# AITRICS/Medical_Tri_Modal_Pilot

Hardware: AMD Instinct MI355X
Metric: tri-modal training samples/s (fwd+bwd+AdamW step, per-GPU batch 64) (higher is better)
Workload: dtype bf16; 1 GPU; BASELINE configs[1]: vslt_img_txt tri_mbt_vsltcls, 6 layers, d_model 256, batch 64/GPU, TIE-len 1000 (N_v=1005), 224x224 CXR, 128-tok text, dropout 0.1, mbt-only-vslt 1, imgtxt-time 1; global_batch=64, parallelism=dp1

## Files before the change

### include/mtmp.h

```cpp
#ifndef MTMP_H
#define MTMP_H
#include <stdint.h>
#ifdef __cplusplus
extern "C" {
#endif

#define MTMP_F32 0
#define MTMP_BF16 1

int mtmp_abi_version(void);
const char* mtmp_last_error(void);

int mtmp_attn_fwd(int dtype, const void* q, const void* k, const void* v, void* o, const void* res, void* o_res,
                  float* lse, const int32_t* kv_len, const float* key_norms, int B, int N, int H, int ld_qkv, int ld_o,
                  float scale, void* stream);
int mtmp_attn_fwd_grouped(int dtype, int n, const void* const* q, const void* const* k, const void* const* v, void* const* o,
                          const void* const* res, void* const* o_res, float* const* lse, const int32_t* const* kv_len,
                          const int32_t* const* row_start, const float* const* key_norms, const int* N, const int* ld_qkv,
                          const int* ld_o, int B, int H, float scale, void* stream);
int mtmp_attn_bwd_grouped(int dtype, int n, const void* const* q, const void* const* k, const void* const* v,
                          const void* const* o, const void* const* d_o, const float* const* lse, const int32_t* const* kv_len,
                          const int32_t* const* row_start, void* const* dq, void* const* dk, void* const* dv,
                          float* const* delta_ws, const int* N, const int* ld_qkv, const int* ld_o, const int* ld_do,
                          const int* ld_dqkv, int B, int H, float scale, void* stream);
int mtmp_attn_cls_fwd(int dtype, const void* q, const void* k, const void* v, int ld_qkv, const void* res, int ld_res, void* o_cls,
                      void* r1_cls, float* lse, const int32_t* kv_len, const int32_t* row_start, int B, int N, int H, int cls_tok,
                      float scale, void* stream);
int mtmp_attn_cls_bwd(int dtype, const void* q, const void* k, const void* v, int ld_qkv, const void* o_cls, const void* d_o,
                      const float* lse, const int32_t* kv_len, const int32_t* row_start, void* dq, void* dk, void* dv, int ld_dqkv,
                      int B, int N, int H, int cls_tok, float scale, void* stream);
long long mtmp_key_norms_floats(long long rows, int H);
int mtmp_key_norms(int dtype, const void* k, float* out, long long rows, int H, int ld, void* stream);

int mtmp_attn_bwd(int dtype, const void* q, const void* k, const void* v, const void* o, const void* d_o,
                  const float* lse, const int32_t* kv_len, void* dq, void* dk, void* dv, float* delta_ws, int B,
                  int N, int H, int ld_qkv, int ld_o, int ld_do, int ld_dqkv, float scale, void* stream);

int mtmp_ln_gemm(int dtype, const void* x, const float* gamma, const float* beta, const void* w, const float* bias,
                 void* y, void* xn, float* stats, int M, int N, int ldx, int ldy, float eps, int relu, float drop_p,
                 unsigned seed, const unsigned* seed_dev, void* stream);

int mtmp_ln_gemm_qkv(int dtype, const void* x, const float* gamma, const float* beta, const void* w, const float* bias,
                     void* y, void* xn, float* stats, float* key_norms, int M, int ldx, float eps, void* stream);

int mtmp_gemm_nt(int dtype, const void* a, const void* w, const float* bias, const void* res, void* y, int M, int N,
                 int K, int lda, int ldy, int ldr, int act, float drop_p, unsigned seed, const unsigned* seed_dev,
                 const void* gate, float gate_scale, const float* row_scale, int rows_per_scale, void* stream);

long long mtmp_sign_bits_bytes(int M, int N);
int mtmp_ln_gemm_signs(int dtype, const void* x, const float* gamma, const float* beta, const void* w, const float* bias,
                       void* y, void* xn, float* stats, int M, int N, int ldx, int ldy, float eps, float drop_p,
                       unsigned seed, const unsigned* seed_dev, void* signs, void* stream);
int mtmp_gemm_nt_signs(int dtype, const void* a, const void* w, void* y, int M, int N, int lda, int ldy,
                       const void* signs, float gate_scale, void* stream);
int mtmp_gemm_nt_signs_drop(int dtype, const void* a, const void* w, void* y, int M, int N, int lda, int ldy,
                            const void* signs, float gate_scale, float drop_p, unsigned seed, const unsigned* seed_dev,
                            void* a_out, void* stream);

long long mtmp_gemm_tn_ws_floats(int M, int N, int K);
int mtmp_gemm_tn(int dtype, const void* dy, const void* x, float* dw, float* db, float* ws, int M, int N, int K,
                 int ldy, int ldx, void* stream);
int mtmp_gemm_tn_live(int dtype, const void* dy, const void* x, float* dw, float* db, float* ws, int M, int N, int K,
                      int ldy, int ldx, const int32_t* rows_live, void* stream);

int mtmp_dropout_bwd(int dtype, const void* g_in, void* g_out, long long n, unsigned seed, const unsigned* seed_dev,
                     float p, void* stream);

int mtmp_ln_bwd_ws_floats(int M);
int mtmp_ln_bwd(int dtype, const void* z, int ldz, const float* stats, const float* gamma, const void* dy,
                const void* d_res, int ldr, void* dz, float* dgamma_dbeta, float* ws, int M, float eps, void* stream);

int mtmp_gemm_lnbwd_ws_floats(int M);
int mtmp_gemm_lnbwd(int dtype, const void* dy, const void* wt, const void* z, int ldz, const float* stats,
                    const float* gamma, const void* d_res, int ldr, void* dz, float* dgamma_dbeta, float* ws, int M,
                    int K, int ldy, float eps, void* stream);

int mtmp_tie_embed_fwd(int dtype, const float* events, const float* params, const float* ftab, void* out, int n,
                       void* stream);
int mtmp_tie_bwd_ws_floats(int n);
int mtmp_tie_embed_bwd(int dtype, const float* events, const float* params, const void* d_out, float* grads,
                       float* ws, int n, void* stream);

int mtmp_time_embed_fwd(int dtype, const float* events, const float* params, const float* ftab, void* out, int n,
// ... 167 lines not shown
```

### medical_tri_modal_pilot_amd/_lib.py

```python
import ctypes
import os
from ctypes import c_char_p, c_float, c_int, c_longlong, c_uint, c_void_p

_HERE = os.path.dirname(os.path.abspath(__file__))
LIB_PATH = os.environ.get("MTMP_LIB", os.path.join(_HERE, "libmtmp_hip.so"))

F32, BF16 = 0, 1

SIGNATURES = {
    "mtmp_abi_version": (c_int, []),
    "mtmp_last_error": (c_char_p, []),
    "mtmp_attn_fwd": (c_int, [c_int] + [c_void_p] * 9 + [c_int] * 5 + [c_float, c_void_p]),
    "mtmp_attn_cls_fwd": (c_int, [c_int] + [c_void_p] * 3 + [c_int, c_void_p, c_int] + [c_void_p] * 5 + [c_int] * 4 + [c_float, c_void_p]),
    "mtmp_attn_cls_bwd": (c_int, [c_int] + [c_void_p] * 3 + [c_int] + [c_void_p] * 8 + [c_int] * 5 + [c_float, c_void_p]),
    "mtmp_attn_fwd_grouped": (c_int, [c_int, c_int] + [c_void_p] * 13 + [c_int, c_int, c_float, c_void_p]),
    "mtmp_attn_bwd_grouped": (c_int, [c_int, c_int] + [c_void_p] * 17 + [c_int, c_int, c_float, c_void_p]),
    "mtmp_key_norms_floats": (c_longlong, [c_longlong, c_int]),
    "mtmp_key_norms": (c_int, [c_int, c_void_p, c_void_p, c_longlong, c_int, c_int, c_void_p]),
    "mtmp_attn_bwd": (c_int, [c_int] + [c_void_p] * 11 + [c_int] * 7 + [c_float, c_void_p]),
    "mtmp_ln_gemm": (c_int, [c_int] + [c_void_p] * 8 + [c_int] * 4 + [c_float, c_int, c_float, c_uint, c_void_p, c_void_p]),
    "mtmp_ln_gemm_qkv": (c_int, [c_int] + [c_void_p] * 9 + [c_int, c_int, c_float, c_void_p]),
    "mtmp_gemm_nt": (c_int, [c_int] + [c_void_p] * 5 + [c_int] * 7 + [c_float, c_uint, c_void_p, c_void_p, c_float, c_void_p, c_int,
                             c_void_p]),
    "mtmp_gemm_nt_live": (c_int, [c_int] + [c_void_p] * 5 + [c_int] * 7 + [c_float, c_uint, c_void_p, c_void_p, c_float, c_void_p, c_int,
                             c_void_p, c_void_p]),
    "mtmp_sign_bits_bytes": (c_longlong, [c_int, c_int]),
    "mtmp_ln_gemm_signs": (c_int, [c_int] + [c_void_p] * 8 + [c_int] * 4 + [c_float, c_float, c_uint, c_void_p, c_void_p, c_void_p]),
    "mtmp_gemm_nt_signs": (c_int, [c_int] + [c_void_p] * 3 + [c_int] * 4 + [c_void_p, c_float, c_void_p]),
    "mtmp_gemm_nt_signs_drop": (c_int, [c_int] + [c_void_p] * 3 + [c_int] * 4 + [c_void_p, c_float, c_float, c_uint, c_void_p,
                                                                                   c_void_p, c_void_p]),
    "mtmp_ln_gemm_qkv_grouped": (c_int, [c_int, c_int] + [c_void_p] * 11 + [c_float, c_void_p, c_void_p]),
    "mtmp_ln_gemm_signs_grouped": (c_int, [c_int, c_int] + [c_void_p] * 10 + [c_int, c_void_p, c_float, c_float, c_void_p, c_void_p,
                                                                                   c_void_p, c_void_p]),
    "mtmp_gemm_nt_grouped": (c_int, [c_int, c_int] + [c_void_p] * 6 + [c_int, c_int] + [c_void_p] * 3 + [c_int, c_float, c_void_p,
                                                                                                       c_void_p, c_void_p, c_void_p]),
    "mtmp_gemm_nt_signs_drop_grouped": (c_int, [c_int, c_int] + [c_void_p] * 4 + [c_int, c_void_p, c_void_p, c_float, c_float,
                                                                                  c_void_p, c_void_p, c_void_p, c_void_p, c_void_p]),
    "mtmp_gemm_lnbwd_grouped": (c_int, [c_int, c_int] + [c_void_p] * 11 + [c_int, c_void_p, c_float, c_void_p, c_void_p]),
    "mtmp_gemm_tn_group_plan": (c_int, [c_int, c_void_p, c_int, c_int, c_void_p]),
    "mtmp_gemm_tn_grouped": (c_int, [c_int, c_int] + [c_void_p] * 4 + [c_int, c_int] + [c_void_p] * 4 + [c_void_p]),
    "mtmp_gemm_tn_slab_rows": (c_int, [c_int] * 4),
    "mtmp_gemm_lnbwd_slab_rows": (c_int, [c_int]),
    "mtmp_reduce_batch": (c_int, [c_void_p] * 6 + [c_int, c_void_p]),
    "mtmp_reduce_scatter": (c_int, [c_void_p] * 5 + [c_int, c_void_p]),
    "mtmp_stream_input_slab_rows": (c_int, [c_int]),
    "mtmp_stream_input_bwd_partials": (c_int, [c_int] + [c_void_p] * 7 + [c_int] * 3 + [c_float, c_uint, c_void_p, c_void_p, c_void_p, c_void_p]),
    "mtmp_stream_input_bwd_grouped": (c_int, [c_int, c_int] + [c_void_p] * 18),
    "mtmp_stream_input_fwd_add": (c_int, [c_int] + [c_void_p] * 8 + [c_int] * 3 + [c_float, c_float, c_uint, c_void_p, c_void_p, c_void_p, c_void_p, c_int, c_void_p]),
    "mtmp_token_sums": (c_int, [c_int, c_int] + [c_void_p] * 5),
    "mtmp_tie_bwd_slab_rows": (c_int, [c_int]),
    "mtmp_tie_time_embed_bwd_partials": (c_int, [c_int, c_void_p, c_int, c_void_p, c_int, c_int] + [c_void_p] * 6),
    "mtmp_publish_scalar": (c_int, [c_void_p, c_void_p, c_void_p]),
    "mtmp_copy_batch": (c_int, [c_void_p] * 4 + [c_int, c_void_p]),
    "mtmp_stream_lengths": (c_int, [c_void_p] * 4 + [c_int] * 3 + [c_void_p]),
    "mtmp_row_starts": (c_int, [c_void_p, c_void_p, c_int, c_int, c_void_p]),
    "mtmp_image_slots": (c_int, [c_void_p, c_int, c_void_p, c_int, c_int, c_void_p]),
    "mtmp_transpose_batch": (c_int, [c_int, c_void_p, c_void_p, c_void_p, c_void_p, c_int, c_void_p]),
    "mtmp_layernorm_rows": (c_int, [c_int] + [c_void_p] * 4 + [c_longlong, c_int, c_float, c_int, c_int, c_int, c_void_p]),
    "mtmp_layernorm_rows_live": (c_int, [c_int] + [c_void_p] * 4 + [c_longlong, c_int, c_float, c_int, c_int, c_int, c_void_p, c_void_p]),
    "mtmp_swin_window_attn": (c_int, [c_int] + [c_void_p] * 3 + [c_int] * 6 + [c_float, c_void_p]),
    "mtmp_swin_window_attn_live": (c_int, [c_int] + [c_void_p] * 3 + [c_int] * 6 + [c_float, c_void_p, c_void_p]),
    "mtmp_layernorm_rows_bwd_slab_rows": (c_int, [c_longlong, c_int]),
    "mtmp_layernorm_rows_bwd": (c_int, [c_int] + [c_void_p] * 5 + [c_longlong, c_int, c_float, c_void_p]),
    "mtmp_gelu_fwd": (c_int, [c_int, c_void_p, c_void_p, c_longlong, c_void_p]),
    "mtmp_gelu_bwd": (c_int, [c_int, c_void_p, c_void_p, c_void_p, c_longlong, c_void_p]),
    "mtmp_swin_window_attn_bwd": (c_int, [c_int] + [c_void_p] * 5 + [c_int] * 6 + [c_float, c_void_p]),
    "mtmp_swin_window_attn_pad": (c_int, [c_int] + [c_void_p] * 4 + [c_int] * 6 + [c_float, c_void_p, c_void_p]),
# ... 68 lines not shown
```

### medical_tri_modal_pilot_amd/ops.py

```python
import contextlib
import ctypes
from typing import Optional

import torch

from . import _lib, tuning
from ._lib import BF16, F32, call

LN_EPS = 1e-6
N_HEAD, D_MODEL, D_HEAD = 4, 256, 64


def _dt(t: torch.Tensor) -> int:
    if t.dtype == torch.float32:
        return F32
    if t.dtype == torch.bfloat16:
        return BF16
    raise TypeError(f"libmtmp_hip kernels take float32 or bfloat16, got {t.dtype}")


def _p(t: Optional[torch.Tensor], byte_offset: int = 0):
    return None if t is None else ctypes.c_void_p(t.data_ptr() + byte_offset)


# ... 1218 lines not shown
        dqkv = attn_bwd(qkv, o, dr1.view(B, N, D), lse, kv_len).view(M, 3 * D)
    else:
        dqkv = attn_bwd_grouped([qkv], [o], [_packed_full(dr1, B, N)], [lse], [kv_len], [pack])[0].view(M, 3 * D)[:live]
    dwqkv, dbqkv = gemm_tn(dqkv, xn1, out=(sink.wqkv, sink.bqkv) if direct else None, defer=red)
    dz, dg1, db1 = gemm_lnbwd(dqkv, wqkvt, z.view(M, D)[:live], st1, g1, d_res2d=dr1, gb_out=sink.gb1 if direct else None, defer=red)
    if late is not None and red:
        late.append((red, sink if direct else None))
    else:
        if red:
            reduce_batch(red)
        if direct:
            sink.flat.mark_ready(sink.idx)
    dz = dz.view(B, N, D) if pack is None else _packed_full(dz, B, N)
    if direct:
        return dz, None
    grads = (dg1, db1, dwqkv[:D], dbqkv[:D], dwqkv[D:2 * D], dbqkv[D:2 * D], dwqkv[2 * D:], dbqkv[2 * D:],
             dg2, db2, dw1, dc1, dw2, dc2)
    return dz, grads


def attn_cls_fwd(qkv, z, kv_len, pack, cls_tok):
    _gpu(qkv, z)
    B, N, _ = qkv.shape
    es = qkv.element_size()
    o = torch.empty(B, D_MODEL, dtype=qkv.dtype, device=qkv.device)
    r1 = torch.empty_like(o)
    lse = torch.empty(B, N_HEAD, dtype=torch.float32, device=qkv.device)
    call("mtmp_attn_cls_fwd", _dt(qkv), _p(qkv), _p(qkv, D_MODEL * es), _p(qkv, 2 * D_MODEL * es), qkv.stride(1), _p(z), z.stride(1),
         _p(o), _p(r1), _p(lse), _p(kv_len), _p(pack), B, N, N_HEAD, int(cls_tok), D_HEAD ** -0.5, _stream())
    return o, r1, lse


def attn_cls_bwd(qkv, o_cls, d_o, lse, kv_len, pack, cls_tok):
    _gpu(qkv, o_cls, d_o)
    B, N, _ = qkv.shape
    es = qkv.element_size()
    dqkv = torch.empty_like(qkv)
    call("mtmp_attn_cls_bwd", _dt(qkv), _p(qkv), _p(qkv, D_MODEL * es), _p(qkv, 2 * D_MODEL * es), qkv.stride(1), _p(o_cls), _p(_c(d_o)),
         _p(lse), _p(kv_len), _p(pack), _p(dqkv), _p(dqkv, D_MODEL * es), _p(dqkv, 2 * D_MODEL * es), dqkv.stride(1), B, N, N_HEAD,
         int(cls_tok), D_HEAD ** -0.5, _stream())
    return dqkv


_cls_rows_cache = {}


def _cls_rows(B, N, cls_tok, dev):
    key = (B, N, cls_tok, dev.type, dev.index)
    if key not in _cls_rows_cache:
        _cls_rows_cache[key] = (torch.arange(B, dtype=torch.int64) * N + cls_tok).to(dev)
    return _cls_rows_cache[key]


def cls_layer_forward(z, kv_len, P, fused, drop_p, seeds, pack, cls_tok):
    B, N, D = z.shape
    g1, b1, g2, b2, c1, c2 = P[0], P[1], P[8], P[9], P[11], P[13]
    wqkv, bqkv, w1c, w2c, w2t, wqkvt, w1t = fused
    z2 = z.view(B * N, D)
    if pack is not None:
        qkv, xn1, st1 = (t[0] for t in ln_gemm_qkv_grouped([z2], [g1], [b1], [wqkv], [bqkv], [pack])[:3])
    else:
        qkv, xn1, st1 = ln_gemm(z2, g1, b1, wqkv, bqkv, 3 * D)
    qkv = qkv.view(B, N, 3 * D)
    o_cls, r1, lse = attn_cls_fwd(qkv, z, kv_len, pack, cls_tok)
    h, xn2, st2, hsign = ln_gemm(r1, g2, b2, w1c, c1, 4 * D, relu=True, drop_p=drop_p, seed=seeds[0], want_signs=True)
    out = gemm_nt(h, w2c, c2, res2d=r1, drop_p=drop_p, seed=seeds[1])
    rows = pack[:B] if pack is not None else _cls_rows(B, N, cls_tok, z.device)
    return out, (z, kv_len, g1, g2, wqkvt, w1t, w2t, xn1, st1, qkv, o_cls, lse, r1, xn2, st2, h, drop_p, seeds, hsign, pack, rows, cls_tok)


def cls_layer_backward(saved, d_cls, sink=None, late=None):
    z, kv_len, g1, g2, wqkvt, w1t, w2t, xn1, st1, qkv, o_cls, lse, r1, xn2, st2, h, p, seeds, hsign, pack, rows, cls_tok = saved
    B, N, D = z.shape
    M = B * N
    d_out = _c(d_cls).to(z.dtype)
    direct = sink is not None and sink.usable()
    red = [] if tuning.DEFER_REDUCTIONS else None
    if hsign is not None and p > 0 and tuning.FOLD_DROPOUT_BWD:
        dh, dy2 = gemm_nt_signs(d_out, w2t, hsign, 1.0 / (1.0 - p), drop_p=p, seed=seeds[1])
    else:
        dy2 = dropout_bwd(d_out, seeds[1], p) if p > 0 else d_out
        dh = gemm_nt_signs(dy2, w2t, hsign, 1.0 / (1.0 - p)) if hsign is not None else gemm_nt(dy2, w2t, gate=h, gate_scale=1.0 / (1.0 - p))
    dw2, dc2 = gemm_tn(dy2, h, out=(sink.w2, sink.c2) if direct else None, defer=red)
    dw1, dc1 = gemm_tn(dh, xn2, out=(sink.w1, sink.c1) if direct else None, defer=red)
    dr1, dg2, db2 = gemm_lnbwd(dh, w1t, r1, st2, g2, d_res2d=d_out, gb_out=sink.gb2 if direct else None, defer=red)
    dqkv = attn_cls_bwd(qkv, o_cls, dr1, lse, kv_len, pack, cls_tok).view(M, 3 * D)
    z2 = z.view(M, D)
    if pack is not None:
        dwqkv, dbqkv = gemm_tn_grouped([dqkv], [xn1], [(sink.wqkv, sink.bqkv) if direct else None], [red], [pack])[0]
        dz, dg1, db1 = gemm_lnbwd_grouped([dqkv], [wqkvt], [z2], [st1], [g1], [None], [sink.gb1 if direct else None], [red], [pack])[0]
    else:
        dwqkv, dbqkv = gemm_tn(dqkv, xn1, out=(sink.wqkv, sink.bqkv) if direct else None, defer=red)
        dz, dg1, db1 = gemm_lnbwd(dqkv, wqkvt, z2, st1, g1, d_res2d=None, gb_out=sink.gb1 if direct else None, defer=red)
    (dz[cls_tok:] if pack is not None else dz).index_add_(0, rows, dr1)
    if late is not None and red:
        late.append((red, sink if direct else None))
    else:
        if red:
            reduce_batch(red)
        if direct:
            sink.flat.mark_ready(sink.idx)
    if direct:
        return dz.view(B, N, D), None
    grads = (dg1, db1, dwqkv[:D], dbqkv[:D], dwqkv[D:2 * D], dbqkv[D:2 * D], dwqkv[2 * D:], dbqkv[2 * D:],
             dg2, db2, dw1, dc1, dw2, dc2)
    return dz.view(B, N, D), grads




def grouped_ok(z) -> bool:
    return tuning.GROUPED_LAUNCHES and z.dtype == torch.bfloat16


def layer_forward_grouped(zs, kv_lens, Ps, fuseds, drop_p, seeds, packs=None, ffn_rows=None):
    n = len(zs)
    B, D = zs[0].shape[0], D_MODEL
    Ns = [z.shape[1] for z in zs]
    packs = [None] * n if packs is None else list(packs)
    z2 = [z.view(B * N, D) for z, N in zip(zs, Ns)]
    qkv, xn1, st1, knorm = ln_gemm_qkv_grouped(z2, [P[0] for P in Ps], [P[1] for P in Ps], [f[0] for f in fuseds], [f[1] for f in fuseds],
                                               packs)
    qkv = [q.view(B, N, 3 * D) for q, N in zip(qkv, Ns)]
    o, r1, lse = attn_fwd_grouped(qkv, kv_lens, list(zs), knorm, packs)
    R = ffn_rows
    if R is not None:
        if any(pk is not None for pk in packs) or any(N < R for N in Ns):
            raise ValueError("ffn_rows: padded streams of at least that many rows")
        r1_2 = [r[:, :R].reshape(B * R, D) for r in r1]
    else:
        r1_2 = [r.view(B * N, D) for r, N in zip(r1, Ns)]
    h, xn2, st2, hsign = ln_gemm_signs_grouped(r1_2, [P[8] for P in Ps], [P[9] for P in Ps], [f[2] for f in fuseds],
                                               [P[11] for P in Ps], 4 * D, drop_p, [sd[0] for sd in seeds], packs)
    out = gemm_nt_grouped(h, [f[3] for f in fuseds], [P[13] for P in Ps], r1_2, drop_p, [sd[1] for sd in seeds], packs)
    if R is not None:
        full = [torch.zeros(B, N, D, dtype=zs[0].dtype, device=zs[0].device) for N in Ns]
        for f_, o_ in zip(full, out):
            f_[:, :R] = o_.view(B, R, D)
        out = full
    saved = [(zs[i], kv_lens[i], Ps[i][0], Ps[i][8], fuseds[i][5], fuseds[i][6], fuseds[i][4], xn1[i], st1[i], qkv[i], o[i], lse[i],
              r1_2[i] if R is not None else r1[i], xn2[i], st2[i], h[i], drop_p, seeds[i], hsign[i], packs[i], R) for i in range(n)]
    return [out[i].view(B, Ns[i], D) for i in range(n)], saved


def layer_backward_grouped(saveds, d_outs, sinks, late):
    n = len(saveds)
    B, D = saveds[0][0].shape[0], D_MODEL
    Ns = [sv[0].shape[1] for sv in saveds]
    Ms = [B * N for N in Ns]
    p = saveds[0][16]
    d_out = [d.view(M, D) for d, M in zip(d_outs, Ms)]
    direct = [sk is not None and sk.usable() for sk in sinks]
    reds = [[] for _ in range(n)]
    col = lambda k: [sv[k] for sv in saveds]
    z, g1, g2, wqkvt, w1t, w2t, xn1, st1, qkv, o, lse, r1, xn2, st2, h, hsign = (col(0), col(2), col(3), col(4), col(5), col(6), col(7),
                                                                              col(8), col(9), col(10), col(11), col(12), col(13),
                                                                              col(14), col(15), col(18))
    kv = col(1)
    seeds = col(17)
# ... 328 lines not shown
```

### medical_tri_modal_pilot_amd/tuning.py

```python

FOLD_DROPOUT_BWD = True
DEFER_REDUCTIONS = True
LATE_REDUCTIONS = False
GROUPED_LAUNCHES = True
GROUP_MODE = "small"
FFN_ROWS_BEFORE_LAST = True
STREAM_ISSUE_ORDER_FWD = (0, 1, 2)
STREAM_ISSUE_ORDER_BWD = (0, 1, 2)
PREFORK_IMAGE_ENCODER = True
INPUT_NODE_ORDER = "long_last"
FUSED_INPUT_TAIL = True
```

Baseline: 8433 samples/s.

## Replace CLS-layer QKV GEMM with algebraic per-row LN score kernels

Result: no change. 8519 samples/s, median of 6 (+1.0%).

```diff
diff --git a/include/mtmp.h b/include/mtmp.h
--- a/include/mtmp.h
+++ b/include/mtmp.h
@@ -29,6 +29,15 @@
 int mtmp_attn_cls_bwd(int dtype, const void* q, const void* k, const void* v, int ld_qkv, const void* o_cls, const void* d_o,
                       const float* lse, const int32_t* kv_len, const int32_t* row_start, void* dq, void* dk, void* dv, int ld_dqkv,
                       int B, int N, int H, int cls_tok, float scale, void* stream);
+int mtmp_cls_ln_rows_chunk(void);
+long long mtmp_cls_ln_rows_floats(int what, int B, int N);
+int mtmp_cls_ln_rows_fwd(const void* z, const float* gamma, const float* beta, const void* wqkv, const float* bqkv,
+                         const int32_t* kv_len, const int32_t* row_start, float* scores, float* stats, float* keep, float* ws,
+                         void* o_cls, void* r1_cls, int B, int N, int cls_tok, float eps, float scale, void* stream);
+int mtmp_cls_ln_rows_bwd(const void* z, const float* gamma, const float* beta, const void* wqkv, const float* bqkv,
+                         const int32_t* kv_len, const int32_t* row_start, const float* scores, const float* stats,
+                         const float* keep, const void* d_o, void* dz, float* ws, float* slab, float* dwqkv, float* dbqkv, int B,
+                         int N, int cls_tok, float eps, float scale, void* stream);
 long long mtmp_key_norms_floats(long long rows, int H);
 int mtmp_key_norms(int dtype, const void* k, float* out, long long rows, int H, int ld, void* stream);
 
diff --git a/medical_tri_modal_pilot_amd/_lib.py b/medical_tri_modal_pilot_amd/_lib.py
--- a/medical_tri_modal_pilot_amd/_lib.py
+++ b/medical_tri_modal_pilot_amd/_lib.py
@@ -13,6 +13,10 @@
     "mtmp_attn_fwd": (c_int, [c_int] + [c_void_p] * 9 + [c_int] * 5 + [c_float, c_void_p]),
     "mtmp_attn_cls_fwd": (c_int, [c_int] + [c_void_p] * 3 + [c_int, c_void_p, c_int] + [c_void_p] * 5 + [c_int] * 4 + [c_float, c_void_p]),
     "mtmp_attn_cls_bwd": (c_int, [c_int] + [c_void_p] * 3 + [c_int] + [c_void_p] * 8 + [c_int] * 5 + [c_float, c_void_p]),
+    "mtmp_cls_ln_rows_chunk": (c_int, []),
+    "mtmp_cls_ln_rows_floats": (c_longlong, [c_int, c_int, c_int]),
+    "mtmp_cls_ln_rows_fwd": (c_int, [c_void_p] * 13 + [c_int] * 3 + [c_float, c_float, c_void_p]),
+    "mtmp_cls_ln_rows_bwd": (c_int, [c_void_p] * 16 + [c_int] * 3 + [c_float, c_float, c_void_p]),
     "mtmp_attn_fwd_grouped": (c_int, [c_int, c_int] + [c_void_p] * 13 + [c_int, c_int, c_float, c_void_p]),
     "mtmp_attn_bwd_grouped": (c_int, [c_int, c_int] + [c_void_p] * 17 + [c_int, c_int, c_float, c_void_p]),
     "mtmp_key_norms_floats": (c_longlong, [c_longlong, c_int]),
diff --git a/medical_tri_modal_pilot_amd/csrc/cls_ln_rows.hip b/medical_tri_modal_pilot_amd/csrc/cls_ln_rows.hip
--- /dev/null
+++ b/medical_tri_modal_pilot_amd/csrc/cls_ln_rows.hip
@@ -0,0 +1,475 @@
+#include "common.hip.h"
+
+namespace {
+constexpr int D = 256, NH = 4, DH = 64;
+constexpr int CR = 64;
+constexpr float LOG2E = 1.4426950408889634f, LN2 = 0.6931471805599453f;
+constexpr int K_XC = 0, K_Q = 256, K_U = 512, K_AB = 1536, K_O = 2560, K_LSE = 2816, K_C = 2820, KEEP = 2824;
+constexpr int W_G = 0, W_DPC = 1024, W_DXC = 1028, W_U = 1284, W_M = 2052, W_S = 3076, WB = 3080;
+
+struct ClsRowsArgs {
+    const bf16* z; const float* gamma; const float* beta; const bf16* wqkv; const float* bqkv;
+    const int* kv_len; const int* row_start;
+    float* scores; float* stats; float* keep;
+    float* pm; float* pa;
+    bf16* o_cls; bf16* r1_cls;
+    const bf16* d_o; bf16* dz; float* wsb;
+    float* mp; float* sp; float* slab;
+    float* dw; float* db;
+    int B, N, NC, cls_tok;
+    float eps, scale;
+};
+
+struct Geo { int row0, kvl, nrows; bool has_cls, uniform; };
+MTMP_DEV Geo geo(const ClsRowsArgs& p, int b) {
+    Geo g;
+    const int kv_raw = p.kv_len ? p.kv_len[b] : p.N;
+    g.has_cls = !(p.row_start && kv_raw <= p.cls_tok);
+    g.uniform = kv_raw <= 0;
+    g.kvl = g.uniform ? p.N : min(kv_raw, p.N);
+    g.nrows = p.row_start ? max(0, min(kv_raw, p.N)) : p.N;
+    g.row0 = p.row_start ? p.row_start[b] : b * p.N;
+    return g;
+}
+
+MTMP_DEV float block_sum(float v, float* red) {
+    v = wave_sum(v);
+    __syncthreads();
+    if ((threadIdx.x & 63) == 0) red[threadIdx.x >> 6] = v;
+    __syncthreads();
+    return (red[0] + red[1]) + (red[2] + red[3]);
+}
+MTMP_DEV float dot4(const f32x4& a, const float (&b)[4]) { return fmaf(a[3], b[3], fmaf(a[2], b[2], fmaf(a[1], b[1], a[0] * b[0]))); }
+
+MTMP_DEV float row_dot(const bf16* w, const float* v) {
+    float a0 = 0.f, a1 = 0.f;
+#pragma unroll 4
+    for (int c = 0; c < D / 8; ++c) {
+        const f32x4 x = load4<bf16>(w + 8 * c), y = load4<bf16>(w + 8 * c + 4);
+#pragma unroll
+        for (int j = 0; j < 4; ++j) { a0 = fmaf(x[j], v[8 * c + j], a0); a1 = fmaf(y[j], v[8 * c + 4 + j], a1); }
+    }
+    return a0 + a1;
+}
+MTMP_DEV float col_dot64(const bf16* w, int r0, const float* v) {
+    float a0 = 0.f, a1 = 0.f;
+    const bf16* col = w + (size_t)r0 * D + threadIdx.x;
+#pragma unroll 8
+    for (int d = 0; d < DH; d += 2) {
+        a0 = fmaf(to_f32(col[(size_t)d * D]), v[d], a0);
+        a1 = fmaf(to_f32(col[(size_t)(d + 1) * D]), v[d + 1], a1);
+    }
+    return a0 + a1;
+}
+
+__global__ __launch_bounds__(256) void cls_rows_fwd_pre_kernel(ClsRowsArgs p) {
+    __shared__ float sx[D], sq[D], red[4];
+    const int b = blockIdx.x, tid = threadIdx.x, lane = tid & 63, wave = tid >> 6;
+    const Geo g = geo(p, b);
+    float* keep = p.keep + (size_t)b * KEEP;
+    if (!g.has_cls) {
+        for (int i = tid; i < KEEP; i += 256) keep[i] = 0.f;
+        return;
+    }
+    const float x = to_f32(p.z[(size_t)(g.row0 + p.cls_tok) * D + tid]);
+    const float mean = block_sum(x, red) * (1.0f / 256.0f);
+    const float d = x - mean;
+    const float sigma = sqrtf(block_sum(d * d, red) * (1.0f / 255.0f));
+    const float rs = 1.0f / (sigma + p.eps);
+    const float xh = fmaf(p.gamma[tid], d * rs, p.beta[tid]);
+    sx[tid] = xh;
+    keep[K_XC + tid] = xh;
+    __syncthreads();
+    const float q = row_dot(p.wqkv + (size_t)tid * D, sx) + p.bqkv[tid];
+    sq[tid] = q;
+    keep[K_Q + tid] = q;
+    __syncthreads();
+    const float c2 = g.uniform ? 0.f : p.scale * LOG2E;
+#pragma unroll
+    for (int h = 0; h < NH; ++h) keep[K_U + h * D + tid] = c2 * col_dot64(p.wqkv, D + h * DH, sq + h * DH);
+    const float cb = wave_sum(sq[wave * DH + lane] * p.bqkv[D + wave * DH + lane]);
+    if (lane == 0) keep[K_C + wave] = c2 * cb;
+}
+
+__global__ __launch_bounds__(256) void cls_rows_fwd_kernel(ClsRowsArgs p) {
+    __shared__ __attribute__((aligned(16))) float sa[4 * NH * D];
+    __shared__ float sm[4 * NH], sl[4 * NH];
+    const int c = blockIdx.x, b = blockIdx.y, tid = threadIdx.x, lane = tid & 63, wave = tid >> 6;
+    const Geo g = geo(p, b);
+    if (!g.has_cls || c * CR >= g.kvl) return;
+    const float* keep = p.keep + (size_t)b * KEEP;
+    const f32x4 gm = ld4f(p.gamma + 4 * lane), bt = ld4f(p.beta + 4 * lane);
+    f32x4 u[NH], a[NH];
+    float ch[NH], m[NH], l[NH];
+#pragma unroll
+    for (int h = 0; h < NH; ++h) {
+        u[h] = ld4f(keep + K_U + h * D + 4 * lane);
+        ch[h] = keep[K_C + h];
+        a[h] = f32x4{0.f, 0.f, 0.f, 0.f};
+        m[h] = -INFINITY;
+        l[h] = 0.f;
+    }
+    const int rbeg = c * CR + wave * 16, rend = min(rbeg + 16, min((c + 1) * CR, g.kvl));
+    for (int r0 = rbeg; r0 < rend; r0 += 4) {
+        f32x4 zv[4];
+#pragma unroll
+        for (int k = 0; k < 4; ++k) zv[k] = load4<bf16>(p.z + (size_t)(g.row0 + min(r0 + k, rend - 1)) * D + 4 * lane);
+#pragma unroll
+        for (int k = 0; k < 4; ++k) {
+            if (r0 + k >= rend) break;
+            const float mean = wave_sum((zv[k][0] + zv[k][1]) + (zv[k][2] + zv[k][3])) * (1.0f / 256.0f);
+            float dd[4], xh[4], s2 = 0.f;
+#pragma unroll
+            for (int i = 0; i < 4; ++i) { dd[i] = zv[k][i] - mean; s2 = fmaf(dd[i], dd[i], s2); }
+            const float sigma = sqrtf(wave_sum(s2) * (1.0f / 255.0f));
+            const float rs = 1.0f / (sigma + p.eps);
+#pragma unroll
+            for (int i = 0; i < 4; ++i) xh[i] = fmaf(gm[i], dd[i] * rs, bt[i]);
+            float s[NH];
+#pragma unroll
+            for (int h = 0; h < NH; ++h) s[h] = wave_sum(dot4(u[h], xh)) + ch[h];
+            const size_t grow = (size_t)(g.row0 + r0 + k);
+            if (lane == 0) {
+                *reinterpret_cast<f32x2*>(p.stats + 2 * grow) = f32x2{mean, rs};
+                *reinterpret_cast<f32x4*>(p.scores + 4 * grow) = f32x4{s[0], s[1], s[2], s[3]};
+            }
+#pragma unroll
+            for (int h = 0; h < NH; ++h) {
+                const float mn = fmaxf(m[h], s[h]);
+                const float al = fast_exp2(m[h] - mn), e = fast_exp2(s[h] - mn);
+                l[h] = fmaf(l[h], al, e);
+#pragma unroll
+                for (int i = 0; i < 4; ++i) a[h][i] = fmaf(a[h][i], al, e * xh[i]);
+                m[h] = mn;
+            }
+        }
+    }
+#pragma unroll
+    for (int h = 0; h < NH; ++h) *reinterpret_cast<f32x4*>(sa + (wave * NH + h) * D + 4 * lane) = a[h];
+    if (lane == 0) {
+#pragma unroll
+        for (int h = 0; h < NH; ++h) { sm[wave * NH + h] = m[h]; sl[wave * NH + h] = l[h]; }
+    }
+    __syncthreads();
+    const size_t pc = (size_t)b * p.NC + c;
+#pragma unroll
+    for (int h = 0; h < NH; ++h) {
+        const float M = fmaxf(fmaxf(sm[h], sm[NH + h]), fmaxf(sm[2 * NH + h], sm[3 * NH + h]));
+        float L = 0.f, A = 0.f;
+#pragma unroll
+        for (int w = 0; w < 4; ++w) {
+            const float f = fast_exp2(sm[w * NH + h] - M);
+            L = fmaf(sl[w * NH + h], f, L);
+            A = fmaf(sa[(w * NH + h) * D + tid], f, A);
+        }
+        p.pa[(pc * NH + h) * D + tid] = A;
+        if (tid == 0) *reinterpret_cast<f32x2*>(p.pm + (pc * NH + h) * 2) = f32x2{M, L};
+    }
+}
+
+__global__ __launch_bounds__(256) void cls_rows_fwd_close_kernel(ClsRowsArgs p) {
+    __shared__ float sab[NH * D];
+    const int b = blockIdx.x, tid = threadIdx.x;
+    const Geo g = geo(p, b);
+    if (!g.has_cls) {
+        p.o_cls[(size_t)b * D + tid] = from_f32<bf16>(0.f);
+        p.r1_cls[(size_t)b * D + tid] = from_f32<bf16>(0.f);
+        return;
+    }
+    float* keep = p.keep + (size_t)b * KEEP;
+    const int nc = (g.kvl + CR - 1) / CR;
+#pragma unroll
+    for (int h = 0; h < NH; ++h) {
+        const float* pm = p.pm + ((size_t)b * p.NC * NH + h) * 2;
+        const float* pa = p.pa + ((size_t)b * p.NC * NH + h) * D + tid;
+        float M = -INFINITY;
+        for (int c = 0; c < nc; ++c) M = fmaxf(M, pm[(size_t)c * NH * 2]);
+        float L = 0.f, A = 0.f;
+        for (int c = 0; c < nc; ++c) {
+            const float f = fast_exp2(pm[(size_t)c * NH * 2] - M);
+            L = fmaf(pm[(size_t)c * NH * 2 + 1], f, L);
+            A = fmaf(pa[(size_t)c * NH * D], f, A);
+        }
+        const float ab = A / L;
+        sab[h * D + tid] = ab;
+        keep[K_AB + h * D + tid] = ab;
+        if (tid == 0) keep[K_LSE + h] = M + log2f(L);
+    }
+    __syncthreads();
+    const int h = tid >> 6;
+    const float o = row_dot(p.wqkv + (size_t)(2 * D + tid) * D, sab + h * D) + p.bqkv[2 * D + tid];
+    keep[K_O + tid] = o;
+    const bf16 ot = from_f32<bf16>(o);
+    p.o_cls[(size_t)b * D + tid] = ot;
+    p.r1_cls[(size_t)b * D + tid] = from_f32<bf16>(to_f32(ot) + to_f32(p.z[(size_t)(g.row0 + p.cls_tok) * D + tid]));
+}
+
+__global__ __launch_bounds__(256) void cls_rows_bwd_pre_kernel(ClsRowsArgs p) {
+    __shared__ float sdo[D];
+    const int b = blockIdx.x, tid = threadIdx.x, lane = tid & 63, wave = tid >> 6;
+    const Geo g = geo(p, b);
+    float* wsb = p.wsb + (size_t)b * WB;
+    if (!g.has_cls) {
+        for (int i = tid; i < WB; i += 256) wsb[i] = 0.f;
+        return;
+    }
+    const float* keep = p.keep + (size_t)b * KEEP;
+    const float dO = to_f32(p.d_o[(size_t)b * D + tid]);
+    sdo[tid] = dO;
+    wsb[W_U + 2 * D + tid] = dO;
+    wsb[W_U + D + tid] = p.scale * keep[K_Q + tid];
+    __syncthreads();
+#pragma unroll
+    for (int h = 0; h < NH; ++h) wsb[W_G + h * D + tid] = col_dot64(p.wqkv, 2 * D + h * DH, sdo + h * DH);
+    const float v = sdo[wave * DH + lane];
+    const float e1 = wave_sum(v * p.bqkv[2 * D + wave * DH + lane]), e2 = wave_sum(v * keep[K_O + wave * DH + lane]);
+    if (lane == 0) wsb[W_DPC + wave] = e1 - e2;
+}
+
+__global__ __launch_bounds__(256) void cls_rows_bwd_kernel(ClsRowsArgs p) {
+    __shared__ __attribute__((aligned(16))) float sred[4 * 6 * D];
+    __shared__ float ssd[4 * NH];
+    const int c = blockIdx.x, b = blockIdx.y, tid = threadIdx.x, lane = tid & 63, wave = tid >> 6;
+    const Geo g = geo(p, b);
+    const size_t wg = (size_t)b * p.NC + c;
+    float* slab = p.slab + wg * 512;
+    const int rows_end = min((c + 1) * CR, g.nrows);
+    if (c * CR >= g.nrows || !g.has_cls) {
+        slab[tid] = 0.f;
+        slab[256 + tid] = 0.f;
+        for (int r = c * CR + wave; r < rows_end; r += 4) store4<bf16>(p.dz + (size_t)(g.row0 + r) * D + 4 * lane, 0.f, 0.f, 0.f, 0.f);
+        return;
+    }
+    const float* keep = p.keep + (size_t)b * KEEP;
+    float* wsb = p.wsb + (size_t)b * WB;
+    const f32x4 gm = ld4f(p.gamma + 4 * lane), bt = ld4f(p.beta + 4 * lane);
+    f32x4 u[NH], gv[NH], mh[NH];
+    float lse[NH], dpc[NH], sds[NH];
+#pragma unroll
+    for (int h = 0; h < NH; ++h) {
+        u[h] = ld4f(keep + K_U + h * D + 4 * lane) * LN2;
+        gv[h] = ld4f(wsb + W_G + h * D + 4 * lane);
+        lse[h] = keep[K_LSE + h];
+        dpc[h] = wsb[W_DPC + h];
+        mh[h] = f32x4{0.f, 0.f, 0.f, 0.f};
+        sds[h] = 0.f;
+    }
+    float part[2][4] = {{0.f, 0.f, 0.f, 0.f}, {0.f, 0.f, 0.f, 0.f}};
+    const int rbeg = c * CR + wave * 16, rend = min(rbeg + 16, rows_end);
+    for (int r0 = rbeg; r0 < rend; r0 += 4) {
+        f32x4 zv[4], sc[4];
+        float mu[4], rs[4];
+#pragma unroll
+        for (int k = 0; k < 4; ++k) {
+            const int row = min(r0 + k, rend - 1);
+            const size_t grow = (size_t)(g.row0 + row);
+            const size_t srow = (size_t)(g.row0 + min(row, g.kvl - 1));
+            zv[k] = load4<bf16>(p.z + grow * D + 4 * lane);
+            sc[k] = ld4f(p.scores + 4 * srow);
+            mu[k] = p.stats[2 * srow];
+            rs[k] = p.stats[2 * srow + 1];
+        }
+#pragma unroll
+        for (int k = 0; k < 4; ++k) {
+            const int row = r0 + k;
+            if (row >= rend) break;
+            const size_t grow = (size_t)(g.row0 + row);
+            if (row >= g.kvl) {
+                if (row == p.cls_tok) *reinterpret_cast<f32x4*>(wsb + W_DXC + 4 * lane) = f32x4{0.f, 0.f, 0.f, 0.f};
+                else store4<bf16>(p.dz + grow * D + 4 * lane, 0.f, 0.f, 0.f, 0.f);
+                continue;
+            }
+            float xn[4], xh[4], dv[4] = {0.f, 0.f, 0.f, 0.f};
+#pragma unroll
+            for (int i = 0; i < 4; ++i) { xn[i] = (zv[k][i] - mu[k]) * rs[k]; xh[i] = fmaf(gm[i], xn[i], bt[i]); }
+#pragma unroll
+            for (int h = 0; h < NH; ++h) {
+                const float pk = fast_exp2(sc[k][h] - lse[h]);
+                const float dP = wave_sum(dot4(gv[h], xh)) + dpc[h];
+                const float ds = g.uniform ? 0.f : pk * dP;
+                sds[h] += ds;
+#pragma unroll
+                for (int i = 0; i < 4; ++i) {
+                    dv[i] = fmaf(pk, gv[h][i], fmaf(ds, u[h][i], dv[i]));
+                    mh[h][i] = fmaf(ds, xh[i], mh[h][i]);
+                }
+            }
+#pragma unroll
+            for (int i = 0; i < 4; ++i) { part[0][i] = fmaf(dv[i], xn[i], part[0][i]); part[1][i] += dv[i]; }
+            if (row == p.cls_tok) {
+                *reinterpret_cast<f32x4*>(wsb + W_DXC + 4 * lane) = f32x4{dv[0], dv[1], dv[2], dv[3]};
+                continue;
+            }
+            float gg[4], sg = 0.f, sgx = 0.f;
+#pragma unroll
+            for (int i = 0; i < 4; ++i) { gg[i] = dv[i] * gm[i]; sg += gg[i]; sgx = fmaf(gg[i], xn[i], sgx); }
+            wave_sum2(sg, sgx);
+            const float sigma = 1.0f / rs[k] - p.eps;
+            const float mg = sg * (1.0f / 256), kx = sgx / (255.0f * sigma);
+            store4<bf16>(p.dz + grow * D + 4 * lane, (gg[0] - mg) * rs[k] - xn[0] * kx, (gg[1] - mg) * rs[k] - xn[1] * kx,
+                         (gg[2] - mg) * rs[k] - xn[2] * kx, (gg[3] - mg) * rs[k] - xn[3] * kx);
+        }
+    }
+    *reinterpret_cast<f32x4*>(sred + (wave * 6 + 0) * D + 4 * lane) = f32x4{part[0][0], part[0][1], part[0][2], part[0][3]};
+    *reinterpret_cast<f32x4*>(sred + (wave * 6 + 1) * D + 4 * lane) = f32x4{part[1][0], part[1][1], part[1][2], part[1][3]};
+#pragma unroll
+    for (int h = 0; h < NH; ++h) *reinterpret_cast<f32x4*>(sred + (wave * 6 + 2 + h) * D + 4 * lane) = mh[h];
+    if (lane == 0) {
+#pragma unroll
+        for (int h = 0; h < NH; ++h) ssd[wave * NH + h] = sds[h];
+    }
+    __syncthreads();
+    for (int i = tid; i < 6 * D; i += 256) {
+        const float s = ((sred[i] + sred[6 * D + i]) + sred[12 * D + i]) + sred[18 * D + i];
+        if (i < 2 * D) slab[i] = s;
+        else p.mp[wg * NH * D + (i - 2 * D)] = s;
+    }
+    if (tid < NH) p.sp[wg * NH + tid] = ((ssd[tid] + ssd[NH + tid]) + ssd[2 * NH + tid]) + ssd[3 * NH + tid];
+}
+
+__global__ __launch_bounds__(256) void cls_rows_bwd_close_kernel(ClsRowsArgs p) {
+    __shared__ float smh[NH * D], sdq[D], sS[NH], red[4];
+    const int b = blockIdx.x, tid = threadIdx.x;
+    const Geo g = geo(p, b);
+    float* slab = p.slab + ((size_t)p.B * p.NC + b) * 512;
+    if (!g.has_cls) {
+        slab[tid] = 0.f;
+        slab[256 + tid] = 0.f;
+        return;
+    }
+    float* wsb = p.wsb + (size_t)b * WB;
+    const int nc = (g.kvl + CR - 1) / CR;
+#pragma unroll
+    for (int h = 0; h < NH; ++h) {
+        const float* mp = p.mp + ((size_t)b * p.NC * NH + h) * D + tid;
+        float s = 0.f;
+        for (int c = 0; c < nc; ++c) s += mp[(size_t)c * NH * D];
+        smh[h * D + tid] = s;
+        wsb[W_M + h * D + tid] = s;
+    }
+    if (tid < NH) {
+        float s = 0.f;
+        for (int c = 0; c < nc; ++c) s += p.sp[((size_t)b * p.NC + c) * NH + tid];
+        sS[tid] = s;
+        wsb[W_S + tid] = s;
+    }
+    __syncthreads();
+    const int h = tid >> 6;
+    const float dq = p.scale * (row_dot(p.wqkv + (size_t)(D + tid) * D, smh + h * D) + p.bqkv[D + tid] * sS[h]);
+    sdq[tid] = dq;
+    wsb[W_U + tid] = dq;
+    __syncthreads();
+    float e = 0.f;
+#pragma unroll
+    for (int h4 = 0; h4 < NH; ++h4) e += col_dot64(p.wqkv, h4 * DH, sdq + h4 * DH);
+    const size_t crow = (size_t)(g.row0 + p.cls_tok);
+    const float x = to_f32(p.z[crow * D + tid]);
+    const float mean = block_sum(x, red) * (1.0f / 256.0f);
+    const float d = x - mean;
+    const float sigma = sqrtf(block_sum(d * d, red) * (1.0f / 255.0f));
+    const float rs = 1.0f / (sigma + p.eps);
+    const float xn = d * rs;
+    const float dv = wsb[W_DXC + tid] + e;
+    const float gg = dv * p.gamma[tid];
+    const float sg = block_sum(gg, red), sgx = block_sum(gg * xn, red);
+    const float mg = sg * (1.0f / 256), kx = sgx / (255.0f * sigma);
+    p.dz[crow * D + tid] = from_f32<bf16>((gg - mg) * rs - xn * kx + to_f32(p.d_o[(size_t)b * D + tid]));
+    slab[tid] = e * xn;
+    slab[256 + tid] = e;
+}
+
+__global__ __launch_bounds__(256) void cls_rows_dw_kernel(ClsRowsArgs p) {
+    __shared__ __attribute__((aligned(16))) float sacc[4 * 8 * D];
+    const int n0 = blockIdx.x * 8, tid = threadIdx.x, cq = tid & 63, bg = tid >> 6;
+    const int part = n0 / D, h = (n0 % D) / DH;
+    f32x4 acc[8];
+#pragma unroll
+    for (int j = 0; j < 8; ++j) acc[j] = f32x4{0.f, 0.f, 0.f, 0.f};
+#pragma unroll 4
+    for (int b = bg; b < p.B; b += 4) {
+        const float* wsb = p.wsb + (size_t)b * WB;
+        const float* keep = p.keep + (size_t)b * KEEP;
+        const float* vp = part == 0 ? keep + K_XC : part == 1 ? wsb + W_M + h * D : keep + K_AB + h * D;
+        const f32x4 v = ld4f(vp + 4 * cq);
+        const f32x4 ua = ld4f(wsb + W_U + n0), ub = ld4f(wsb + W_U + n0 + 4);
+#pragma unroll
+        for (int j = 0; j < 4; ++j) { acc[j] += ua[j] * v; acc[4 + j] += ub[j] * v; }
+    }
+#pragma unroll
+    for (int j = 0; j < 8; ++j) *reinterpret_cast<f32x4*>(sacc + (bg * 8 + j) * D + 4 * cq) = acc[j];
+    __syncthreads();
+    for (int i = tid; i < 8 * D; i += 256)
+        p.dw[(size_t)n0 * D + i] = ((sacc[i] + sacc[8 * D + i]) + sacc[16 * D + i]) + sacc[24 * D + i];
+    if (tid < 8) {
+        float s = 0.f;
+        for (int b = 0; b < p.B; ++b) {
+            const float* wsb = p.wsb + (size_t)b * WB;
+            s = fmaf(wsb[W_U + n0 + tid], part == 1 ? wsb[W_S + h] : 1.0f, s);
+        }
+        p.db[n0 + tid] = s;
+    }
+}
+
+bool cls_rows_ok(int B, int N, int cls_tok) { return B > 0 && B <= 65535 && N > 0 && N <= 65536 && cls_tok >= 0 && cls_tok < N; }
+}
+
+extern "C" int mtmp_cls_ln_rows_chunk(void) { return CR; }
+
+extern "C" long long mtmp_cls_ln_rows_floats(int what, int B, int N) {
+    if (B <= 0 || N <= 0) return 0;
+    const long long nc = (N + CR - 1) / CR;
+    switch (what) {
+    case 0: return (long long)B * KEEP;
+    case 1: return (long long)B * nc * NH * (2 + D);
+    case 2: return (long long)B * WB + (long long)B * nc * NH * (D + 1);
+    case 3: return (long long)B * nc + B;
+    default: return 0;
+    }
+}
+
+extern "C" int mtmp_cls_ln_rows_fwd(const void* z, const float* gamma, const float* beta, const void* wqkv, const float* bqkv,
+                                    const int32_t* kv_len, const int32_t* row_start, float* scores, float* stats, float* keep,
+                                    float* ws, void* o_cls, void* r1_cls, int B, int N, int cls_tok, float eps, float scale,
+                                    void* stream) {
+    MTMP_CHECK_ARG(z && gamma && beta && wqkv && bqkv && scores && stats && keep && ws && o_cls && r1_cls,
+                   "mtmp_cls_ln_rows_fwd: null pointer");
+    MTMP_CHECK_ARG(cls_rows_ok(B, N, cls_tok) && (!row_start || kv_len), "mtmp_cls_ln_rows_fwd: bad argument (B=%d N=%d cls=%d)", B, N,
+                   cls_tok);
+    hipStream_t st = (hipStream_t)stream;
+    ClsRowsArgs a{};
+    a.z = (const bf16*)z; a.gamma = gamma; a.beta = beta; a.wqkv = (const bf16*)wqkv; a.bqkv = bqkv;
+    a.kv_len = kv_len; a.row_start = row_start; a.scores = scores; a.stats = stats; a.keep = keep;
+    a.B = B; a.N = N; a.NC = (N + CR - 1) / CR; a.cls_tok = cls_tok; a.eps = eps; a.scale = scale;
+    a.pm = ws; a.pa = ws + (size_t)B * a.NC * NH * 2;
+    a.o_cls = (bf16*)o_cls; a.r1_cls = (bf16*)r1_cls;
+    hipLaunchKernelGGL(cls_rows_fwd_pre_kernel, dim3(B), dim3(256), 0, st, a);
+    hipLaunchKernelGGL(cls_rows_fwd_kernel, dim3(a.NC, B), dim3(256), 0, st, a);
+    hipLaunchKernelGGL(cls_rows_fwd_close_kernel, dim3(B), dim3(256), 0, st, a);
+    MTMP_CHECK_LAUNCH("mtmp_cls_ln_rows_fwd");
+    return MTMP_OK;
+}
+
+extern "C" int mtmp_cls_ln_rows_bwd(const void* z, const float* gamma, const float* beta, const void* wqkv, const float* bqkv,
+                                    const int32_t* kv_len, const int32_t* row_start, const float* scores, const float* stats,
+                                    const float* keep, const void* d_o, void* dz, float* ws, float* slab, float* dwqkv,
+                                    float* dbqkv, int B, int N, int cls_tok, float eps, float scale, void* stream) {
+    MTMP_CHECK_ARG(z && gamma && beta && wqkv && bqkv && scores && stats && keep && d_o && dz && ws && slab && dwqkv && dbqkv,
+                   "mtmp_cls_ln_rows_bwd: null pointer");
+    MTMP_CHECK_ARG(cls_rows_ok(B, N, cls_tok) && (!row_start || kv_len), "mtmp_cls_ln_rows_bwd: bad argument (B=%d N=%d cls=%d)", B, N,
+                   cls_tok);
+    hipStream_t st = (hipStream_t)stream;
+    ClsRowsArgs a{};
+    a.z = (const bf16*)z; a.gamma = gamma; a.beta = beta; a.wqkv = (const bf16*)wqkv; a.bqkv = bqkv;
+    a.kv_len = kv_len; a.row_start = row_start; a.scores = const_cast<float*>(scores); a.stats = const_cast<float*>(stats);
+    a.keep = const_cast<float*>(keep);
+    a.B = B; a.N = N; a.NC = (N + CR - 1) / CR; a.cls_tok = cls_tok; a.eps = eps; a.scale = scale;
+    a.d_o = (const bf16*)d_o; a.dz = (bf16*)dz; a.wsb = ws;
+    a.mp = ws + (size_t)B * WB; a.sp = a.mp + (size_t)B * a.NC * NH * D;
+    a.slab = slab; a.dw = dwqkv; a.db = dbqkv;
+    hipLaunchKernelGGL(cls_rows_bwd_pre_kernel, dim3(B), dim3(256), 0, st, a);
+    hipLaunchKernelGGL(cls_rows_bwd_kernel, dim3(a.NC, B), dim3(256), 0, st, a);
+    hipLaunchKernelGGL(cls_rows_bwd_close_kernel, dim3(B), dim3(256), 0, st, a);
+    hipLaunchKernelGGL(cls_rows_dw_kernel, dim3(3 * D / 8), dim3(256), 0, st, a);
+    MTMP_CHECK_LAUNCH("mtmp_cls_ln_rows_bwd");
+    return MTMP_OK;
+}
diff --git a/medical_tri_modal_pilot_amd/ops.py b/medical_tri_modal_pilot_amd/ops.py
--- a/medical_tri_modal_pilot_amd/ops.py
+++ b/medical_tri_modal_pilot_amd/ops.py
@@ -1294,10 +1294,50 @@
     return _cls_rows_cache[key]
 
 
+def _cls_rows_buf(what, B, N, dev):
+    return torch.empty(_lib.lib().mtmp_cls_ln_rows_floats(what, B, N), dtype=torch.float32, device=dev)
+
+
+def cls_ln_rows_fwd(z, kv_len, g1, b1, wqkv, bqkv, pack, cls_tok):
+    _gpu(z, wqkv)
+    B, N, D = z.shape
+    dev = z.device
+    scores = torch.empty(B * N, N_HEAD, dtype=torch.float32, device=dev)
+    stats = torch.empty(B * N, 2, dtype=torch.float32, device=dev)
+    keep, ws = _cls_rows_buf(0, B, N, dev), _cls_rows_buf(1, B, N, dev)
+    o = torch.empty(B, D, dtype=z.dtype, device=dev)
+    r1 = torch.empty_like(o)
+    with kernel_marks("cls_ln_rows_fwd", B * N):
+        call("mtmp_cls_ln_rows_fwd", _p(z), _p(g1), _p(b1), _p(wqkv), _p(bqkv), _p(kv_len), _p(pack), _p(scores), _p(stats), _p(keep),
+             _p(ws), _p(o), _p(r1), B, N, int(cls_tok), LN_EPS, D_HEAD ** -0.5, _stream())
+    return o, r1, (scores, stats, keep)
+
+
+def cls_ln_rows_bwd(z, kv_len, g1, b1, wqkv, bqkv, pack, cls_tok, kept, d_o, dwqkv, dbqkv):
+    _gpu(z, d_o)
+    B, N, D = z.shape
+    dev = z.device
+    scores, stats, keep = kept
+    dz = torch.empty(B * N, D, dtype=z.dtype, device=dev)
+    rows = _lib.lib().mtmp_cls_ln_rows_floats(3, B, N)
+    slab = torch.empty(rows, 2 * D, dtype=torch.float32, device=dev)
+    ws = _cls_rows_buf(2, B, N, dev)
+    with kernel_marks("cls_ln_rows_bwd", B * N):
+        call("mtmp_cls_ln_rows_bwd", _p(z), _p(g1), _p(b1), _p(wqkv), _p(bqkv), _p(kv_len), _p(pack), _p(scores), _p(stats), _p(keep),
+             _p(_c(d_o)), _p(dz), _p(ws), _p(slab), _p(dwqkv), _p(dbqkv), B, N, int(cls_tok), LN_EPS, D_HEAD ** -0.5, _stream())
+    return dz, (slab, rows)
+
+
 def cls_layer_forward(z, kv_len, P, fused, drop_p, seeds, pack, cls_tok):
     B, N, D = z.shape
     g1, b1, g2, b2, c1, c2 = P[0], P[1], P[8], P[9], P[11], P[13]
     wqkv, bqkv, w1c, w2c, w2t, wqkvt, w1t = fused
+    if tuning.CLS_LAYER_LN_ROWS and z.dtype == torch.bfloat16:
+        wqkv = _c(wqkv)
+        o_cls, r1, kept = cls_ln_rows_fwd(z, kv_len, g1, b1, wqkv, bqkv, pack, cls_tok)
+        h, xn2, st2, hsign = ln_gemm(r1, g2, b2, w1c, c1, 4 * D, relu=True, drop_p=drop_p, seed=seeds[0], want_signs=True)
+        out = gemm_nt(h, w2c, c2, res2d=r1, drop_p=drop_p, seed=seeds[1])
+        return out, ("ln_rows", z, kv_len, g1, b1, g2, wqkv, bqkv, w1t, w2t, kept, r1, xn2, st2, h, drop_p, seeds, hsign, pack, cls_tok)
     z2 = z.view(B * N, D)
     if pack is not None:
         qkv, xn1, st1 = (t[0] for t in ln_gemm_qkv_grouped([z2], [g1], [b1], [wqkv], [bqkv], [pack])[:3])
@@ -1312,7 +1352,11 @@
 
 
 def cls_layer_backward(saved, d_cls, sink=None, late=None):
-    z, kv_len, g1, g2, wqkvt, w1t, w2t, xn1, st1, qkv, o_cls, lse, r1, xn2, st2, h, p, seeds, hsign, pack, rows, cls_tok = saved
+    ln_rows = saved[0] == "ln_rows" if isinstance(saved[0], str) else False
+    if ln_rows:
+        _, z, kv_len, g1, b1, g2, wqkv, bqkv, w1t, w2t, kept, r1, xn2, st2, h, p, seeds, hsign, pack, cls_tok = saved
+    else:
+        z, kv_len, g1, g2, wqkvt, w1t, w2t, xn1, st1, qkv, o_cls, lse, r1, xn2, st2, h, p, seeds, hsign, pack, rows, cls_tok = saved
     B, N, D = z.shape
     M = B * N
     d_out = _c(d_cls).to(z.dtype)
@@ -1326,6 +1370,22 @@
     dw2, dc2 = gemm_tn(dy2, h, out=(sink.w2, sink.c2) if direct else None, defer=red)
     dw1, dc1 = gemm_tn(dh, xn2, out=(sink.w1, sink.c1) if direct else None, defer=red)
     dr1, dg2, db2 = gemm_lnbwd(dh, w1t, r1, st2, g2, d_res2d=d_out, gb_out=sink.gb2 if direct else None, defer=red)
+    if ln_rows:
+        if direct:
+            dwqkv, dbqkv, gb = sink.wqkv, sink.bqkv, sink.gb1
+        else:
+            dwqkv = torch.empty(3 * D, D, dtype=torch.float32, device=z.device)
+            dbqkv = torch.empty(3 * D, dtype=torch.float32, device=z.device)
+            gb = torch.empty(2 * D, dtype=torch.float32, device=z.device)
+        dz, (slab, srows) = cls_ln_rows_bwd(z, kv_len, g1, b1, wqkv, bqkv, pack, cls_tok, kept, dr1, dwqkv, dbqkv)
+        entry = (slab, srows, 2 * D, gb, 2 * D, None)
+        if red is not None:
+            red.append(entry)
+        else:
+            reduce_batch([entry])
+        dg1, db1 = gb[:D], gb[D:]
+        return _cls_layer_backward_tail(dz.view(B, N, D), red, late, direct, sink,
+                                        (dg1, db1, dwqkv, dbqkv, dg2, db2, dw1, dc1, dw2, dc2))
     dqkv = attn_cls_bwd(qkv, o_cls, dr1, lse, kv_len, pack, cls_tok).view(M, 3 * D)
     z2 = z.view(M, D)
     if pack is not None:
@@ -1335,6 +1395,10 @@
         dwqkv, dbqkv = gemm_tn(dqkv, xn1, out=(sink.wqkv, sink.bqkv) if direct else None, defer=red)
         dz, dg1, db1 = gemm_lnbwd(dqkv, wqkvt, z2, st1, g1, d_res2d=None, gb_out=sink.gb1 if direct else None, defer=red)
     (dz[cls_tok:] if pack is not None else dz).index_add_(0, rows, dr1)
+    return _cls_layer_backward_tail(dz.view(B, N, D), red, late, direct, sink, (dg1, db1, dwqkv, dbqkv, dg2, db2, dw1, dc1, dw2, dc2))
+
+
+def _cls_layer_backward_tail(dz, red, late, direct, sink, g):
     if late is not None and red:
         late.append((red, sink if direct else None))
     else:
@@ -1343,10 +1407,12 @@
         if direct:
             sink.flat.mark_ready(sink.idx)
     if direct:
-        return dz.view(B, N, D), None
+        return dz, None
+    dg1, db1, dwqkv, dbqkv, dg2, db2, dw1, dc1, dw2, dc2 = g
+    D = D_MODEL
     grads = (dg1, db1, dwqkv[:D], dbqkv[:D], dwqkv[D:2 * D], dbqkv[D:2 * D], dwqkv[2 * D:], dbqkv[2 * D:],
              dg2, db2, dw1, dc1, dw2, dc2)
-    return dz.view(B, N, D), grads
+    return dz, grads
 
 
 
diff --git a/medical_tri_modal_pilot_amd/tuning.py b/medical_tri_modal_pilot_amd/tuning.py
--- a/medical_tri_modal_pilot_amd/tuning.py
+++ b/medical_tri_modal_pilot_amd/tuning.py
@@ -10,3 +10,4 @@
 PREFORK_IMAGE_ENCODER = True
 INPUT_NODE_ORDER = "long_last"
 FUSED_INPUT_TAIL = True
+CLS_LAYER_LN_ROWS = True
```
